# dyustc/CTC-Attention-Mispronunciation

Measured on AMD Instinct MI355X. Metric: phoneme-frames/sec joint CTC-attn decode, 41-phone vocab, higher is better.
Workload: dtype f32 -- reference width (operands with all 24 significand bits, fp32 accumulate; see `accuracy`: closer to a float64 evaluation than ATen's own fp32): the large time-batched contractions (conv0/conv1, BiLSTM and text input projections) run on the bf16 matrix cores as f32x6 = each fp32 operand as thre

## Files before the change

ctc-attention-mispronunciation_amd/csrc/api.hip:

```cpp
#include <stdarg.h>
#include <stdio.h>
#include <string.h>

#include <algorithm>
#include <cmath>
#include <mutex>
#include <vector>

#include "mdd_internal.h"

namespace mdd {

static thread_local char g_err[512] = "";

void set_error(const char *fmt, ...) {
    va_list ap;
    va_start(ap, fmt);
    vsnprintf(g_err, sizeof(g_err), fmt, ap);
    va_end(ap);
}

struct DeviceGate {
    std::mutex mu;
    hipEvent_t done = nullptr;
    hipStream_t stream = nullptr;
    bool armed = false;
};
static DeviceGate g_gate[64];

struct DevBuf {
    float *p = nullptr;
    size_t cap = 0;
};

struct GraphKey {
    const void *x, *x1, *out, *tlen, *llen;
    int B, T, L, Traw;
    bool operator<(const GraphKey &o) const { return memcmp(this, &o, sizeof(GraphKey)) < 0; }
};

}

struct mdd_model {
    mdd_config cfg;
    int device = 0;
    bool finalized = false, taps = false, use_graph = true;
    int precision = 2;
    std::map<std::string, std::vector<float>> host;
    float *w_conv0 = nullptr, *sc0 = nullptr, *sh0 = nullptr;
    float *w_conv1t = nullptr, *sc1 = nullptr, *sh1 = nullptr;
    std::vector<float *> wih, whh, bn_scale, bn_shift;
    float *emb = nullptr, *t_wih = nullptr, *t_whh = nullptr, *t_bias = nullptr;
    float *w_score = nullptr, *fscale = nullptr, *fshift = nullptr, *w_fc = nullptr, *w_fcp = nullptr;
    std::vector<mdd::SplitPtr> wih_s, whh_s;
    std::vector<unsigned short *> wih_3;
    unsigned short *t_wih_3 = nullptr, *w_conv1_3 = nullptr;
    std::vector<unsigned short *> whh_3;
    unsigned short *t_whh_3 = nullptr;
    mdd::SplitPtr t_whh_s{nullptr, nullptr};
    mdd::SplitPtr t_wih_s{nullptr, nullptr}, w_score_s{nullptr, nullptr}, w_conv1_s{nullptr, nullptr};
    std::vector<void *> owned;
    mdd::DevBuf y0, seq0, gx, act[2], xraw, hbuf, cbuf, embo, text, key, S;
    mdd::DevBuf seq0_s, act_s[2], x_s, embo_s, text_s, key_s, hsplit, hx;
    mdd::DevBuf p3;
    std::vector<mdd::DevBuf> tap_rnn;
    int *err_flag = nullptr;
    hipStream_t cap_stream = nullptr;
    int lastB = 0, lastT = 0, lastL = 0;
    int raw_T = 0;
    const int *tlen = nullptr, *llen = nullptr;
    mdd::DevBuf xstack;
    std::map<mdd::GraphKey, hipGraphExec_t> graphs;
    int W1() const { return (cfg.feat + 2 - 3) / 2 + 1; }
    int W2() const { return (W1() + 2 - 3) / 2 + 1; }
    int rnn_in() const { return cfg.channels * W2(); }
    int granule_max_b = 1024;
    bool lstm_persist = true;
    int n_cu = 0;
    unsigned int *sync_words = nullptr;
    bool lstm_x3 = false;
    bool conv_fused() const { return (x3() || x6()) && cfg.feat == 243 && cfg.channels == 32; }
    bool packed_h() const { return cfg.hidden == 384 || cfg.hidden == 256; }
    bool persist(int B) const { return lstm_persist && !lstm_x3 && packed_h() && B <= granule_max_b && (x3() || lstm_persist_f32); }
    bool lstm_persist_f32 = true;
    bool lstm_persist_x6 = true;
    bool lstm_x6_force = false;
    bool lx6(int B) const {
        return x6() && lstm_persist_x6 && persist(B) && B <= mdd::lstm_x6_max_b(cfg.hidden) && (lstm_x6_force || cfg.hidden == 384 || B <= 128);
    }
    bool x6() const {
        return precision == 2 && rnn_in() % 32 == 0 && (2 * cfg.hidden) % 32 == 0 && cfg.emb_dim % 32 == 0;
    }
    bool x3() const {
        return precision == 1 && (cfg.hidden == 384 || cfg.hidden == 256) && rnn_in() % 32 == 0 && cfg.emb_dim % 32 == 0;
    }
};

namespace mdd {

static int upload(mdd_model *m, const std::vector<float> &h, float **dev) {
    MDD_HIP_CHECK(hipMalloc((void **)dev, h.size() * sizeof(float)));
    m->owned.push_back(*dev);
    MDD_HIP_CHECK(hipMemcpy(*dev, h.data(), h.size() * sizeof(float), hipMemcpyHostToDevice));
    return MDD_OK;
}

static unsigned short host_bf16(float x) {
    unsigned u; memcpy(&u, &x, 4);
    u += 0x7FFFu + ((u >> 16) & 1u);
    return (unsigned short)(u >> 16);
}
static float host_bf16_f32(unsigned short b) { unsigned u = (unsigned)b << 16; float f; memcpy(&f, &u, 4); return f; }

static int upload_split(mdd_model *m, const std::vector<float> &h, SplitPtr *out) {
    const size_t n = h.size();
    std::vector<unsigned short> buf(2 * n);
    for (size_t i = 0; i < n; i++) {
        buf[i] = host_bf16(h[i]);
        buf[n + i] = host_bf16(h[i] - host_bf16_f32(buf[i]));
    }
    unsigned short *d = nullptr;
    MDD_HIP_CHECK(hipMalloc((void **)&d, 2 * n * sizeof(unsigned short)));
    m->owned.push_back(d);
    MDD_HIP_CHECK(hipMemcpy(d, buf.data(), 2 * n * sizeof(unsigned short), hipMemcpyHostToDevice));
    out->hi = d; out->lo = d + n;
    return MDD_OK;
}

static SplitPtr split_view(const DevBuf &b, size_t n) {
    SplitPtr s; s.hi = reinterpret_cast<unsigned short *>(b.p); s.lo = s.hi ? s.hi + n : nullptr; return s;
}
static const SplitPtr kNoSplit = {nullptr, nullptr};

static thread_local bool g_ws_moved = false;

static std::mutex g_prep_mu;

static int ensure(DevBuf &b, size_t n, hipStream_t zero_stream) {
    if (b.cap >= n) return MDD_OK;
    g_ws_moved = true;
    if (b.p) MDD_HIP_CHECK(hipFree(b.p));
    b.p = nullptr; b.cap = 0;
    MDD_HIP_CHECK(hipMalloc((void **)&b.p, n * sizeof(float)));
    MDD_HIP_CHECK(hipMemsetAsync(b.p, 0, n * sizeof(float), zero_stream));
    MDD_HIP_CHECK(hipStreamSynchronize(zero_stream));
    b.cap = n;
    return MDD_OK;
}

static const std::vector<float> *get(mdd_model *m, const std::string &key, size_t numel) {
    auto it = m->host.find(key);
    if (it == m->host.end()) { set_error("weight '%s' was never loaded", key.c_str()); return nullptr; }
    if (it->second.size() != numel) {
        set_error("weight '%s' has %zu elements, expected %zu", key.c_str(), it->second.size(), numel);
        return nullptr;
    }
    return &it->second;
}

static bool bn_fold(mdd_model *m, const std::string &prefix, int n, std::vector<float> &scale, std::vector<float> &shift) {
    const auto *w = get(m, prefix + ".weight", n), *b = get(m, prefix + ".bias", n);
    const auto *mu = get(m, prefix + ".running_mean", n), *var = get(m, prefix + ".running_var", n);
    if (!w || !b || !mu || !var) return false;
    scale.resize(n); shift.resize(n);
    for (int i = 0; i < n; i++) {
        scale[i] = (*w)[i] / sqrtf((*var)[i] + m->cfg.bn_eps);
        shift[i] = (*b)[i] - (*mu)[i] * scale[i];
    }
    return true;
}

static bool pack_gate_rows(mdd_model *m, const std::string &base, const char *what, int H, int K, std::vector<float> &out) {
    out.assign((size_t)2 * 4 * H * K, 0.f);
    for (int d = 0; d < 2; d++) {
        const auto *w = get(m, base + what + (d ? "_reverse" : ""), (size_t)4 * H * K);
        if (!w) return false;
        for (int g = 0; g < 4; g++)
            for (int u = 0; u < H; u++)
                memcpy(&out[((size_t)d * 4 * H + u * 4 + g) * K], &(*w)[((size_t)g * H + u) * K], sizeof(float) * K);
    }
    return true;
}

static bool use_packed(const mdd_model *m) { return m->cfg.hidden == 384 || m->cfg.hidden == 256; }

static void pack_whh(const std::vector<float> &w, int H, std::vector<float> &out) {
    const int NUT = H / 4, J = H / 16;
    out.resize(w.size());
    for (int d = 0; d < 2; d++)
        for (int ut = 0; ut < NUT; ut++)
            for (int j = 0; j < J; j++)
                for (int lane = 0; lane < 64; lane++)
                    for (int mm = 0; mm < 4; mm++)
                        out[((((size_t)d * NUT + ut) * J + j) * 64 + lane) * 4 + mm] =
                            w[((size_t)d * 4 * H + ut * 16 + (lane & 15)) * H + 16 * j + 4 * (lane >> 4) + mm];
}

static int upload_split3(mdd_model *m, const std::vector<float> &w, unsigned short **out) {
    const size_t n = w.size();
    std::vector<unsigned short> buf(3 * n);
    for (size_t i = 0; i < n; i++) {
        buf[i] = host_bf16(w[i]);
        const float r1 = w[i] - host_bf16_f32(buf[i]);
        buf[n + i] = host_bf16(r1);
        buf[2 * n + i] = host_bf16(r1 - host_bf16_f32(buf[n + i]));
    }
    MDD_HIP_CHECK(hipMalloc((void **)out, 3 * n * sizeof(unsigned short)));
    m->owned.push_back(*out);
    MDD_HIP_CHECK(hipMemcpy(*out, buf.data(), 3 * n * sizeof(unsigned short), hipMemcpyHostToDevice));
    return MDD_OK;
}

struct Stage { const char *name; int launches; double flops; };

static int n_stages(const mdd_model *m) { return 2 + 2 * m->cfg.layers + 6; }

static int run_stage(mdd_model *m, int si, const float *x, int B, int T, const int64_t *x1, int L, float *logp,
                     hipStream_t st, Stage *info) {
    const mdd_config &c = m->cfg;
    const int H = c.hidden, H2 = 2 * H, G2 = 8 * H, Tp = T / 2, Lp = L, nl = c.layers;
    const bool x3 = m->x3();
    const size_t rows = (size_t)Tp * B, trows = (size_t)L * B;
    static thread_local char namebuf[32];
    Stage dummy; if (!info) info = &dummy;
    info->launches = 1; info->flops = 0.0;
    if (si == 0 && m->conv_fused()) {
        info->name = "conv_fused";
        info->flops = 2.0 * 9 * c.channels * (double)B * Tp * m->W2() * (c.channels + 6.0);
        if (m->x6())
            return launch_conv_fused3(x, m->w_conv0, m->sc0, m->sh0, m->w_conv1_3, m->sc1, m->sh1, reinterpret_cast<unsigned short *>(m->p3.p),
                                      m->taps ? m->seq0.p : nullptr, B, T, m->raw_T, st);
        return launch_conv_fused(x, m->w_conv0, m->sc0, m->sh0, m->w_conv1_s, m->sc1, m->sh1, split_view(m->seq0_s, rows * m->rnn_in()),
                                 nullptr, B, T, m->raw_T, st);
    }
    if (si == 1 && m->conv_fused()) { info->name = "conv1_in_fused"; info->launches = 0; return MDD_OK; }
    if (si == 0) { info->name = "conv0"; info->flops = 2.0 * 9 * c.channels * (double)B * T * m->W1();
        return launch_conv0(x, m->w_conv0, m->sc0, m->sh0, m->y0.p, B, T, c.feat, c.channels, st); }
    if (si == 1) { info->name = "conv1"; info->flops = 2.0 * 9 * c.channels * c.channels * (double)B * Tp * m->W2();
        return launch_conv1(m->y0.p, m->w_conv1t, m->sc1, m->sh1, x3 ? nullptr : m->seq0.p,
                            x3 ? split_view(m->seq0_s, rows * m->rnn_in()) : kNoSplit, B, T, m->W1(), c.channels, st); }
    si -= 2;
    if (si < 2 * nl) {
        const int n = si / 2;
        const int K = n == 0 ? m->rnn_in() : H2;
        if (si % 2 == 0) {
            snprintf(namebuf, sizeof(namebuf), "gemm_ih%d", n); info->name = namebuf;
            info->flops = 2.0 * (double)Tp * B * G2 * K;
            if (x3) {
                const SplitPtr in = n == 0 ? split_view(m->seq0_s, rows * K) : split_view(m->act_s[(n - 1) & 1], rows * K);
                return launch_gemm_bf16x3(in, m->wih_s[n], nullptr, m->gx.p, nullptr, Tp * B, G2, K, K, K, G2, 1, 0, 0, 0, st);
            }
            const float *in = n == 0 ? m->seq0.p : m->act[(n - 1) & 1].p;
            if (m->x6()) {
                unsigned short *p3 = reinterpret_cast<unsigned short *>(m->p3.p);
                if (!(n == 0 && m->conv_fused()))
                    if (int rc = launch_split3(in, Tp * B, K, K, p3, st)) return rc;
                return launch_gemm_f32x6(p3, (size_t)Tp * B * K, m->wih_3[n], (size_t)G2 * K, nullptr, m->gx.p, Tp * B, G2, K, G2, st);
            }
            return launch_gemm_nt(in, m->wih[n], nullptr, m->gx.p, Tp * B, G2, K, K, K, G2, 1, 0, 0, 0, st);
        }
        snprintf(namebuf, sizeof(namebuf), "lstm%d", n); info->name = namebuf;
        info->launches = Tp; info->flops = 2.0 * 2 * (double)B * H * 4 * H * Tp;
        LstmStepArgs a;
        a.gx = m->gx.p; a.whh = m->whh[n]; a.hbuf = m->hbuf.p; a.cbuf = m->cbuf.p;
        a.T = Tp; a.B = B; a.H = H; a.packed = use_packed(m);
        a.whh_split = m->whh_s[n]; a.hsplit = (x3 && m->lstm_x3) ? reinterpret_cast<unsigned short *>(m->hsplit.p) : nullptr;
        a.seqlen = m->tlen;
        if (n == nl - 1) {
            a.out = m->xraw.p; a.out_raw = m->xraw.p; a.oscale = nullptr; a.oshift = nullptr;
            a.out_split = x3 ? split_view(m->x_s, rows * H2) : kNoSplit;
        } else {
            a.out = x3 ? nullptr : m->act[n & 1].p; a.out_raw = m->taps ? m->tap_rnn[n].p : nullptr;
            a.out_split = x3 ? split_view(m->act_s[n & 1], rows * H2) : kNoSplit;
            a.oscale = m->bn_scale[n + 1]; a.oshift = m->bn_shift[n + 1];
        }
        if (m->persist(B)) {
            info->launches = 1;
            if (m->lx6(B)) return launch_lstm_layer_x6(a, m->whh_3[n], reinterpret_cast<unsigned short *>(m->hx.p), m->sync_words, m->err_flag, st);
            return x3 ? launch_lstm_layer_granule(a, reinterpret_cast<unsigned short *>(m->hx.p), m->sync_words, m->err_flag, st)
                      : launch_lstm_layer_f32(a, reinterpret_cast<unsigned short *>(m->hx.p), m->sync_words, m->err_flag, st);
        }
        return launch_lstm_layer(a, st);
    }
    si -= 2 * nl;
    switch (si) {
    case 0:
        info->name = "embed";
        return launch_embed(m->emb, c.emb_rows, c.emb_dim, x1, B, L, x3 ? nullptr : m->embo.p,
                            x3 ? split_view(m->embo_s, trows * c.emb_dim) : kNoSplit, m->err_flag, st);
    case 1:
        info->name = "gemm_text"; info->flops = 2.0 * (double)L * B * G2 * c.emb_dim;
        if (x3) return launch_gemm_bf16x3(split_view(m->embo_s, trows * c.emb_dim), m->t_wih_s, m->t_bias, m->gx.p, nullptr, L * B, G2,
                                          c.emb_dim, c.emb_dim, c.emb_dim, G2, 1, 0, 0, 0, st);
        if (m->x6()) {
            unsigned short *p3 = reinterpret_cast<unsigned short *>(m->p3.p);
            if (int rc = launch_split3(m->embo.p, L * B, c.emb_dim, c.emb_dim, p3, st)) return rc;
            return launch_gemm_f32x6(p3, (size_t)L * B * c.emb_dim, m->t_wih_3, (size_t)G2 * c.emb_dim, m->t_bias, m->gx.p, L * B, G2, c.emb_dim, G2, st);
        }
        return launch_gemm_nt(m->embo.p, m->t_wih, m->t_bias, m->gx.p, L * B, G2, c.emb_dim, c.emb_dim, c.emb_dim, G2, 1, 0, 0, 0, st);
    case 2: {
        info->name = "lstm_text"; info->launches = L; info->flops = 2.0 * 2 * (double)B * H * 4 * H * L;
        LstmStepArgs a;
        a.gx = m->gx.p; a.whh = m->t_whh; a.hbuf = m->hbuf.p; a.cbuf = m->cbuf.p;
        a.out = m->text.p; a.out_raw = m->text.p; a.oscale = nullptr; a.oshift = nullptr;
        a.out_split = x3 ? split_view(m->text_s, trows * H2) : kNoSplit;
        a.T = L; a.B = B; a.H = H; a.packed = use_packed(m);
        a.whh_split = m->t_whh_s; a.hsplit = (x3 && m->lstm_x3) ? reinterpret_cast<unsigned short *>(m->hsplit.p) : nullptr;
        a.seqlen = m->llen;
        if (m->persist(B)) {
            info->launches = 1;
            if (m->lx6(B)) return launch_lstm_layer_x6(a, m->t_whh_3, reinterpret_cast<unsigned short *>(m->hx.p), m->sync_words, m->err_flag, st);
            return x3 ? launch_lstm_layer_granule(a, reinterpret_cast<unsigned short *>(m->hx.p), m->sync_words, m->err_flag, st)
                      : launch_lstm_layer_f32(a, reinterpret_cast<unsigned short *>(m->hx.p), m->sync_words, m->err_flag, st);
        }
// ... 19 lines not shown
}

int device_gate_enter(int device, hipStream_t st, bool *held) {
    *held = false;
    hipStreamCaptureStatus cs = hipStreamCaptureStatusNone;
    if (st && hipStreamIsCapturing(st, &cs) == hipSuccess && cs != hipStreamCaptureStatusNone) return MDD_OK;
    DeviceGate &g = g_gate[device & 63];
    g.mu.lock();
    *held = true;
    if (g.armed && g.stream != st) {
        hipError_t e = hipStreamWaitEvent(st, g.done, 0);
        if (e != hipSuccess) { g.mu.unlock(); *held = false; set_error("device gate: %s", hipGetErrorString(e)); return MDD_ERR_HIP; }
    }
    return MDD_OK;
}
int device_gate_leave(int device, hipStream_t st, bool held, int rc) {
    if (!held) return rc;
    DeviceGate &g = g_gate[device & 63];
    hipError_t e = hipSuccess;
    if (!g.done) e = hipEventCreateWithFlags(&g.done, hipEventDisableTiming);
    if (e == hipSuccess) e = hipEventRecord(g.done, st);
    if (e == hipSuccess) { g.armed = true; g.stream = st; }
    g.mu.unlock();
    if (e != hipSuccess && rc == MDD_OK) { set_error("device gate: %s", hipGetErrorString(e)); return MDD_ERR_HIP; }
    return rc;
}
static int gate_enter(mdd_model *m, hipStream_t st, bool *held) { return device_gate_enter(m->device, st, held); }
static int gate_leave(mdd_model *m, hipStream_t st, bool held, int rc) { return device_gate_leave(m->device, st, held, rc); }

static int forward_enqueue(mdd_model *m, const float *x, int B, int T, const int64_t *x1, int L, float *logp, hipStream_t st) {
    for (int si = 0; si < n_stages(m); si++)
        if (int rc = run_stage(m, si, x, B, T, x1, L, logp, st, nullptr)) return rc;
    return MDD_OK;
}

}

using namespace mdd;

extern "C" const char *mdd_last_error(void) { return g_err; }
extern "C" int mdd_version(void) { return 100; }

extern "C" int mdd_create(const mdd_config *cfg, int device, mdd_model **out) {
    if (!cfg || !out) { set_error("mdd_create: null argument"); return MDD_ERR_ARG; }
    if (cfg->hidden <= 0 || cfg->hidden % 4 || cfg->layers < 1 || cfg->num_class < 2 || cfg->feat < 3 ||
        (cfg->channels != 32 && cfg->channels != 4) || cfg->emb_rows < 1 || cfg->emb_dim < 1) {
        set_error("mdd_create: unsupported geometry (hidden %% 4 == 0, channels in {32,4})");
        return MDD_ERR_ARG;
    }
    int ndev = 0;
    MDD_HIP_CHECK(hipGetDeviceCount(&ndev));
    if (device < 0 || device >= ndev) { set_error("mdd_create: device %d of %d", device, ndev); return MDD_ERR_ARG; }
    MDD_HIP_CHECK(hipSetDevice(device));
    hipDeviceProp_t prop;
    MDD_HIP_CHECK(hipGetDeviceProperties(&prop, device));
    if (strncmp(prop.gcnArchName, "gfx950", 6) != 0) {
        set_error("libmdd_hip is built for gfx950 (MI355X) only; device %d is %s", device, prop.gcnArchName);
        return MDD_ERR_ARG;
    }
    mdd_model *m = new mdd_model();
    m->cfg = *cfg;
    m->device = device;
    const char *pr = getenv("MDD_PRECISION");
    if (pr && (!strcmp(pr, "f32") || !strcmp(pr, "0"))) m->precision = 0;
    if (pr && (!strcmp(pr, "bf16x3") || !strcmp(pr, "1"))) m->precision = 1;
    if (pr && (!strcmp(pr, "f32x6") || !strcmp(pr, "2"))) m->precision = 2;
    const char *lx = getenv("MDD_LSTM");
    m->lstm_x3 = lx && !strcmp(lx, "x3");
    if (lx && !strcmp(lx, "step")) m->lstm_persist = false;
    const char *g = getenv("MDD_GRAPH");
    m->use_graph = !(g && g[0] == '0');
    if (int rc = init_kernel_attributes()) { delete m; return rc; }
    if (int rc = init_lstm_attributes()) { delete m; return rc; }
    if (int rc = init_granule_attributes()) { delete m; return rc; }
    if (int rc = init_lstm_f32_attributes()) { delete m; return rc; }
    if (int rc = init_lstm_x6_attributes()) { delete m; return rc; }
    if (int rc = init_conv_attributes()) { delete m; return rc; }
    if (int rc = init_gemm_attributes()) { delete m; return rc; }
    if (int rc = init_gemm_x6_attributes()) { delete m; return rc; }
    m->n_cu = prop.multiProcessorCount;
    if (!persistent_grid_fits(m->n_cu)) m->lstm_persist = false;
    if (!persistent_f32_grid_fits(m->n_cu)) m->lstm_persist_f32 = false;
    if (!persistent_x6_grid_fits(m->n_cu)) m->lstm_persist_x6 = false;
    { const char *e6 = getenv("MDD_LSTM_X6"); if (e6 && e6[0] == '0') m->lstm_persist_x6 = false; if (e6 && e6[0] == 'f') m->lstm_x6_force = true; }
    hipError_t e = hipMalloc((void **)&m->err_flag, sizeof(int));
    if (e == hipSuccess) e = hipMemset(m->err_flag, 0, sizeof(int));
    if (e == hipSuccess) e = hipStreamCreateWithFlags(&m->cap_stream, hipStreamNonBlocking);
    if (e == hipSuccess) e = hipMalloc((void **)&m->sync_words, 32 * sizeof(unsigned int));
    if (e != hipSuccess) { set_error("mdd_create: %s", hipGetErrorString(e)); delete m; return MDD_ERR_HIP; }
    *out = m;
    return MDD_OK;
}

extern "C" void mdd_destroy(mdd_model *m) {
    if (!m) return;
    (void)hipSetDevice(m->device);
    (void)hipDeviceSynchronize();
    for (auto &kv : m->graphs) (void)hipGraphExecDestroy(kv.second);
    for (void *p : m->owned) (void)hipFree(p);
    DevBuf *bufs[] = {&m->y0, &m->seq0, &m->gx, &m->act[0], &m->act[1], &m->xraw, &m->hbuf, &m->cbuf, &m->embo, &m->text, &m->key, &m->S,
                      &m->seq0_s, &m->act_s[0], &m->act_s[1], &m->x_s, &m->embo_s, &m->text_s, &m->key_s, &m->hsplit, &m->hx, &m->xstack, &m->p3};
    for (DevBuf *b : bufs) if (b->p) (void)hipFree(b->p);
    for (auto &b : m->tap_rnn) if (b.p) (void)hipFree(b.p);
    if (m->err_flag) (void)hipFree(m->err_flag);
    if (m->cap_stream) (void)hipStreamDestroy(m->cap_stream);
    if (m->sync_words) (void)hipFree(m->sync_words);
    delete m;
}

extern "C" int mdd_load_weight(mdd_model *m, const char *key, const float *data, const int64_t *shape, int32_t ndim) {
    if (!m || !key || (!data && ndim > 0) || ndim < 0 || ndim > 4) { set_error("mdd_load_weight: bad argument"); return MDD_ERR_ARG; }
    std::string k(key);
    if (k.size() > 19 && k.compare(k.size() - 19, 19, "num_batches_tracked") == 0) return MDD_OK;
    size_t n = 1;
    for (int i = 0; i < ndim; i++) { if (shape[i] < 0) { set_error("negative dim"); return MDD_ERR_ARG; } n *= (size_t)shape[i]; }
    m->host[k].assign(data, data + n);
    m->finalized = false;
    return MDD_OK;
}

extern "C" int mdd_finalize_weights(mdd_model *m) {
    if (!m) { set_error("null model"); return MDD_ERR_ARG; }
    MDD_HIP_CHECK(hipSetDevice(m->device));
    const mdd_config &c = m->cfg;
    const int ch = c.channels, H = c.hidden;
    int rc;
    for (void *p : m->owned) (void)hipFree(p);
    m->owned.clear(); m->wih.clear(); m->whh.clear(); m->wih_s.clear(); m->whh_s.clear(); m->wih_3.clear(); m->t_wih_3 = nullptr;
    m->bn_scale.assign(c.layers, nullptr); m->bn_shift.assign(c.layers, nullptr);
    for (auto &kv : m->graphs) (void)hipGraphExecDestroy(kv.second);
    m->graphs.clear();
    std::vector<float> sc, sh, tmp;
    {
        const auto *w0 = get(m, "conv.0.conv.weight", (size_t)ch * 9), *b0 = get(m, "conv.0.conv.bias", ch);
        const auto *w1 = get(m, "conv.1.conv.weight", (size_t)ch * ch * 9), *b1 = get(m, "conv.1.conv.bias", ch);
        if (!w0 || !b0 || !w1 || !b1) return MDD_ERR_STATE;
        if (!bn_fold(m, "conv.0.batch_norm", ch, sc, sh)) return MDD_ERR_STATE;
        for (int i = 0; i < ch; i++) sh[i] += (*b0)[i] * sc[i];
        if ((rc = upload(m, *w0, &m->w_conv0)) || (rc = upload(m, sc, &m->sc0)) || (rc = upload(m, sh, &m->sh0))) return rc;
        if (!bn_fold(m, "conv.1.batch_norm", ch, sc, sh)) return MDD_ERR_STATE;
        for (int i = 0; i < ch; i++) sh[i] += (*b1)[i] * sc[i];
        tmp.assign((size_t)ch * 9 * ch, 0.f);
        for (int co = 0; co < ch; co++)
            for (int ci = 0; ci < ch; ci++)
                for (int k = 0; k < 9; k++) tmp[((size_t)ci * 9 + k) * ch + co] = (*w1)[((size_t)co * ch + ci) * 9 + k];
        if ((rc = upload(m, tmp, &m->w_conv1t)) || (rc = upload(m, sc, &m->sc1)) || (rc = upload(m, sh, &m->sh1))) return rc;
        tmp.assign((size_t)ch * 9 * ch, 0.f);
        for (int co = 0; co < ch; co++)
            for (int ci = 0; ci < ch; ci++)
                for (int k = 0; k < 9; k++) tmp[((size_t)co * 9 + k) * ch + ci] = (*w1)[((size_t)co * ch + ci) * 9 + k];
        if ((rc = upload_split(m, tmp, &m->w_conv1_s))) return rc;
        {
            const size_t n = tmp.size();
            std::vector<unsigned short> buf(3 * n);
            for (size_t i = 0; i < n; i++) {
                buf[i] = host_bf16(tmp[i]);
                const float r1 = tmp[i] - host_bf16_f32(buf[i]);
                buf[n + i] = host_bf16(r1);
                buf[2 * n + i] = host_bf16(r1 - host_bf16_f32(buf[n + i]));
            }
            MDD_HIP_CHECK(hipMalloc((void **)&m->w_conv1_3, 3 * n * sizeof(unsigned short)));
            m->owned.push_back(m->w_conv1_3);
            MDD_HIP_CHECK(hipMemcpy(m->w_conv1_3, buf.data(), 3 * n * sizeof(unsigned short), hipMemcpyHostToDevice));
        }
    }
    for (int n = 0; n < c.layers; n++) {
// ... 328 lines not shown
```

ctc-attention-mispronunciation_amd/csrc/frontend.hip:

```cpp
#include "mdd_internal.h"

namespace mdd {

__global__ void stack_skip_kernel(const float *__restrict__ raw, int T_raw, int D, int right, int skip, int kept,
                                  int T_out, float *__restrict__ out) {
    const int W = (right + 1) * D;
    const int b = blockIdx.y, i = blockIdx.x;
    const float *src = raw + (size_t)b * T_raw * D;
    float *dst = out + ((size_t)b * T_out + i) * W;
    for (int j = threadIdx.x; j < W; j += blockDim.x) {
        float v = 0.f;
        if (i < kept) {
            int r = j / D, c = j - r * D;
            int s = i * skip + r;
            if (s > T_raw - 1) s = T_raw - 1;
            v = src[(size_t)s * D + c];
        }
        dst[j] = v;
    }
}

int launch_stack_skip(const float *raw, int B, int T_raw, int D, int right, int skip, int n_down, float *out,
                      hipStream_t st) {
    if (B <= 0 || T_raw <= 0 || D <= 0 || right < 0) { set_error("stack_skip: bad shape"); return MDD_ERR_ARG; }
// ... 259 lines not shown
            }
        }
        __syncthreads();
        f32x16 acc;
#pragma unroll
        for (int r = 0; r < 16; r++) acc[r] = 0.f;
        const int m = min(mt * 32 + li, W2 - 1);
#pragma unroll
        for (int i = 0; i < 9; i++) {
            const int kb = kh2 * 9 + i, kk = kb >> 1, kh = kk / 3, kw = kk - kh * 3;
            const int khs = kh + rot >= 3 ? kh + rot - 3 : kh + rot;
            const int off = (khs * CF_NCOL + 2 * m + kw) * CF_COLB + ((kb & 1) * 16 + half * 8) * 2;
            const bf16x8 ah = *reinterpret_cast<const bf16x8 *>(yh + off);
            const bf16x8 al = *reinterpret_cast<const bf16x8 *>(yl + off);
            if (NP == 3) {
                const bf16x8 am = *reinterpret_cast<const bf16x8 *>(ym + off);
                acc = __builtin_amdgcn_mfma_f32_32x32x16_bf16(am, bwm[i], acc, 0, 0, 0);
                acc = __builtin_amdgcn_mfma_f32_32x32x16_bf16(ah, bwl[i], acc, 0, 0, 0);
                acc = __builtin_amdgcn_mfma_f32_32x32x16_bf16(al, bwh[i], acc, 0, 0, 0);
                acc = __builtin_amdgcn_mfma_f32_32x32x16_bf16(ah, bwm[i], acc, 0, 0, 0);
                acc = __builtin_amdgcn_mfma_f32_32x32x16_bf16(am, bwh[i], acc, 0, 0, 0);
            } else {
                acc = __builtin_amdgcn_mfma_f32_32x32x16_bf16(ah, bwl[i], acc, 0, 0, 0);
                acc = __builtin_amdgcn_mfma_f32_32x32x16_bf16(al, bwh[i], acc, 0, 0, 0);
            }
            acc = __builtin_amdgcn_mfma_f32_32x32x16_bf16(ah, bwh[i], acc, 0, 0, 0);
        }
        if (kh2 == 1) {
#pragma unroll
            for (int r = 0; r < 16; r++) red[mt * 1024 + r * 64 + lane] = acc[r];
        }
        __syncthreads();
        if (kh2 == 0) {
            const float s1 = sc1[li], h1 = sh1[li];
#pragma unroll
            for (int r = 0; r < 16; r++) {
                const int wo = mt * 32 + (r & 3) + 8 * (r >> 2) + 4 * half;
                if (wo < W2) {
                    float v = (acc[r] + red[mt * 1024 + r * 64 + lane]) * s1 + h1;
                    v = v > 0.f ? v : 0.f;
                    __bf16 hb = (__bf16)v;
                    const float r1 = v - (float)hb;
                    oh[li * W2 + wo] = *reinterpret_cast<unsigned short *>(&hb);
                    if (NP == 3) {
                        __bf16 mb = (__bf16)r1, lb = (__bf16)(r1 - (float)mb);
                        om[li * W2 + wo] = *reinterpret_cast<unsigned short *>(&mb);
                        ol[li * W2 + wo] = *reinterpret_cast<unsigned short *>(&lb);
                    } else { __bf16 lb = (__bf16)r1; ol[li * W2 + wo] = *reinterpret_cast<unsigned short *>(&lb); }
                }
            }
        }
        __syncthreads();
        if (NP == 3) {
            const size_t mrows = (size_t)Tp * B;
            if (tid < 244) {
                const size_t dst = (((size_t)(tid >> 2) * mrows + rowid) * 32 + (tid & 3) * 8);
                *reinterpret_cast<u32x4 *>(out_hi + dst) = *reinterpret_cast<const u32x4 *>(oh + tid * 8);
                *reinterpret_cast<u32x4 *>(out_lo + dst) = *reinterpret_cast<const u32x4 *>(om + tid * 8);
                *reinterpret_cast<u32x4 *>(out_lo + mrows * ROW + dst) = *reinterpret_cast<const u32x4 *>(ol + tid * 8);
            }
            if (out_f32)
                for (int i = tid; i < ROW; i += 256)
                    out_f32[(size_t)rowid * ROW + i] = (__uint_as_float((unsigned)oh[i] << 16) + __uint_as_float((unsigned)om[i] << 16)) + __uint_as_float((unsigned)ol[i] << 16);
        } else {
            const size_t base = (size_t)rowid * ROW;
            if (tid < 244) *reinterpret_cast<u32x4 *>(out_hi + base + tid * 8) = *reinterpret_cast<const u32x4 *>(oh + tid * 8);
            else if (tid - 244 < 12) {
                const int q = tid - 244;
                *reinterpret_cast<u32x4 *>(out_lo + base + q * 8) = *reinterpret_cast<const u32x4 *>(ol + q * 8);
            }
            if (tid < 232) {
                const int q = tid + 12;
                *reinterpret_cast<u32x4 *>(out_lo + base + q * 8) = *reinterpret_cast<const u32x4 *>(ol + q * 8);
            }
            if (out_f32)
                for (int i = tid; i < ROW; i += 256)
                    out_f32[base + i] = __uint_as_float((unsigned)oh[i] << 16) + __uint_as_float((unsigned)ol[i] << 16);
        }
    }
}

size_t conv_fused_smem(int np) { return 5 * CF_XLD * 4 + (size_t)np * CF_YPLANE + 2048 * 4 + (size_t)np * 1952 * 2; }

int launch_conv_fused(const float *x, const float *w0, const float *sc0, const float *sh0, SplitPtr w1, const float *sc1,
                      const float *sh1, SplitPtr out, float *out_f32, int B, int T, int Traw, hipStream_t st) {
    const int Tp = T / 2;
    if (Tp <= 0 || B <= 0) return MDD_OK;
    int S = (1024 + B - 1) / B;
    S = S < 1 ? 1 : (S > Tp ? Tp : S);
    const int seg = (Tp + S - 1) / S;
    S = (Tp + seg - 1) / seg;
    hipLaunchKernelGGL(conv_fused_kernel<2>, dim3(B * S), dim3(256), conv_fused_smem(2), st, x, w0, sc0, sh0, w1.hi, w1.lo, sc1, sh1,
                       out.hi, out.lo, out_f32, B, T, Traw, S, seg);
    MDD_LAUNCH_CHECK();
    return MDD_OK;
}

int launch_conv_fused3(const float *x, const float *w0, const float *sc0, const float *sh0, const unsigned short *w1_3, const float *sc1,
                       const float *sh1, unsigned short *out3, float *out_f32, int B, int T, int Traw, hipStream_t st) {
    const int Tp = T / 2;
    if (Tp <= 0 || B <= 0) return MDD_OK;
    int S = (512 + B - 1) / B;
    S = S < 1 ? 1 : (S > Tp ? Tp : S);
    const int seg = (Tp + S - 1) / S;
    S = (Tp + seg - 1) / seg;
    const size_t plane = (size_t)Tp * B * 1952;
    hipLaunchKernelGGL(conv_fused_kernel<3>, dim3(B * S), dim3(256), conv_fused_smem(3), st, x, w0, sc0, sh0, w1_3, w1_3 + 32 * 288, sc1, sh1,
                       out3, out3 + plane, out_f32, B, T, Traw, S, seg);
    MDD_LAUNCH_CHECK();
    return MDD_OK;
}

int init_conv_attributes() {
    MDD_HIP_CHECK(hipFuncSetAttribute((const void *)conv_fused_kernel<2>, hipFuncAttributeMaxDynamicSharedMemorySize, 96 * 1024));
    MDD_HIP_CHECK(hipFuncSetAttribute((const void *)conv_fused_kernel<3>, hipFuncAttributeMaxDynamicSharedMemorySize, 128 * 1024));
    return MDD_OK;
}

}
```

ctc-attention-mispronunciation_amd/csrc/mdd_internal.h:

```cpp
#pragma once
#include <hip/hip_runtime.h>
#include <stdint.h>

#include <map>
#include <string>
#include <vector>

#include "../../include/mdd_hip.h"

namespace mdd {

void set_error(const char *fmt, ...);

#define MDD_HIP_CHECK(expr)                                                                     \
    do {                                                                                        \
        hipError_t e_ = (expr);                                                                 \
        if (e_ != hipSuccess) {                                                                 \
            mdd::set_error("%s failed: %s (%s:%d)", #expr, hipGetErrorString(e_), __FILE__, __LINE__); \
            return MDD_ERR_HIP;                                                                 \
        }                                                                                       \
    } while (0)

#define MDD_LAUNCH_CHECK() MDD_HIP_CHECK(hipGetLastError())

struct SplitPtr { unsigned short *hi, *lo; };

int launch_gemm_nt(const float *A, const float *W, const float *bias, float *C, int M, int N, int K, int lda, int ldw,
                   int ldc, int batch, long sA, long sW, long sC, hipStream_t st);

int launch_gemm_f32(bool ta, bool tb, const float *A, const float *B, const float *bias, float *C, int M, int N, int K, int lda, int ldb,
                    int ldc, int batch, long sA, long sB, long sC, bool accumulate, hipStream_t st, int ksplit = 0);

int launch_gemm_bf16x3(const SplitPtr &A, const SplitPtr &W, const float *bias, float *C, const SplitPtr *Csplit, int M, int N,
                       int K, int lda, int ldw, int ldc, int batch, long sA, long sW, long sC, hipStream_t st);
int init_gemm_attributes();
int launch_split(const float *x, size_t n, const SplitPtr &out, hipStream_t st);
int launch_unsplit(const SplitPtr &in, size_t n, float *x, hipStream_t st);
int launch_split3(const float *x, int rows, int K, int ld, unsigned short *planes, hipStream_t st);
int launch_gemm_f32x6(const unsigned short *A3, size_t a_plane, const unsigned short *W3, size_t w_plane, const float *bias, float *C, int M, int N, int K,
                      int ldc, hipStream_t st, long long *stamps = nullptr);
int init_gemm_x6_attributes();

int launch_stack_skip(const float *raw, int B, int T_raw, int D, int right, int skip, int n_down, float *out,
                      hipStream_t st);
int launch_conv0(const float *x, const float *w, const float *scale, const float *shift, float *y0, int B, int T, int F,
                 int ch, hipStream_t st);
int launch_conv1(const float *y0, const float *w_t, const float *scale, const float *shift, float *seq, SplitPtr seq_split, int B,
                 int T, int W1, int ch, hipStream_t st);

int launch_conv_fused(const float *x, const float *w0, const float *sc0, const float *sh0, SplitPtr w1, const float *sc1,
                      const float *sh1, SplitPtr out, float *out_f32, int B, int T, int Traw, hipStream_t st);
int launch_conv_fused3(const float *x, const float *w0, const float *sc0, const float *sh0, const unsigned short *w1_3, const float *sc1,
                       const float *sh1, unsigned short *out3, float *out_f32, int B, int T, int Traw, hipStream_t st);
int init_conv_attributes();

struct LstmStepArgs {
    const float *gx;
    const float *whh;
    float *hbuf;
    float *cbuf;
    float *out;
    SplitPtr out_split;
    float *out_raw;
    const float *oscale;
    const float *oshift;
    int T, B, H;
    SplitPtr whh_split;
    unsigned short *hsplit;
    int packed;
    float *gates_save = nullptr;
    float *c_save = nullptr;
    const int *seqlen = nullptr;
};
int launch_lstm_layer(const LstmStepArgs &a, hipStream_t st);

int launch_embed(const float *table, int rows, int E, const int64_t *ids, int B, int L, float *out, SplitPtr out_split,
                 int *err_flag, hipStream_t st);
int launch_attn_tail(const float *S, int Lp, const float *X, const float *V, const float *fscale, const float *fshift,
                     const float *wfc, const float *wfcp, float *logp, int Tp, int B, int L, int H2, int C, hipStream_t st,
                     const int *llen = nullptr);

int init_kernel_attributes();
int init_ctc_attributes();
int init_lstm_attributes();
int granule_bg(int B);
int init_granule_attributes();
int persistent_grid_fits(int n_cu);
int launch_lstm_layer_granule(const LstmStepArgs &s, unsigned short *hx, unsigned int *sync, int *err_flag, hipStream_t st);
int launch_zero_fill(void *p, size_t n, hipStream_t st);
int launch_lstm_layer_f32(const LstmStepArgs &s, unsigned short *hx, unsigned int *sync, int *err_flag, hipStream_t st);
int init_lstm_f32_attributes();
int persistent_f32_grid_fits(int n_cu);
int launch_lstm_layer_x6(const LstmStepArgs &s, const unsigned short *whh3, unsigned short *hx, unsigned int *sync, int *err_flag, hipStream_t st);
int init_lstm_x6_attributes();
int persistent_x6_grid_fits(int n_cu);
size_t lstm_x6_hx_bytes(int H, int B);
int lstm_x6_max_b(int H);
size_t lstm_bwd_granule_hx_bytes(int H);
int launch_lstm_bwd_granule(const float *dout, const float *gates, const float *cst, SplitPtr whhT, float *dg, int T, int B, int H, unsigned short *hx,
                            unsigned int *sync, int *err_flag, hipStream_t st);
int device_gate_enter(int device, hipStream_t st, bool *held);
int device_gate_leave(int device, hipStream_t st, bool held, int rc);

}
```

Baseline: 4.188 million.

## Add multi-row fused conv kernel reusing conv0 rows via rotating LDS ring

Adds a new fused conv0+conv1 f32x6 kernel that produces two output time rows per iteration with 512 threads, keeping a rotating ring of conv0 output rows in LDS so overlapping rows are not recomputed. It also prefetches the next input tile into registers while the current tile is computed, and splits the conv1 K reduction across wave groups with an LDS reduction. It becomes the default path for f32x6, with the old row-wise kernel kept behind MDD_CONV=rowwise. The trade-offs are higher LDS and register use with one block per CU, extra barriers, and segment lengths rounded up to a multiple of the row count.

```diff
diff --git a/ctc-attention-mispronunciation_amd/csrc/api.hip b/ctc-attention-mispronunciation_amd/csrc/api.hip
--- a/ctc-attention-mispronunciation_amd/csrc/api.hip
+++ b/ctc-attention-mispronunciation_amd/csrc/api.hip
@@ -85,6 +85,7 @@
     bool lstm_persist_f32 = true;
     bool lstm_persist_x6 = true;
     bool lstm_x6_force = false;
+    bool conv_rowwise = false;
     bool lx6(int B) const {
         return x6() && lstm_persist_x6 && persist(B) && B <= mdd::lstm_x6_max_b(cfg.hidden) && (lstm_x6_force || cfg.hidden == 384 || B <= 128);
     }
@@ -229,7 +230,7 @@
         info->flops = 2.0 * 9 * c.channels * (double)B * Tp * m->W2() * (c.channels + 6.0);
         if (m->x6())
             return launch_conv_fused3(x, m->w_conv0, m->sc0, m->sh0, m->w_conv1_3, m->sc1, m->sh1, reinterpret_cast<unsigned short *>(m->p3.p),
-                                      m->taps ? m->seq0.p : nullptr, B, T, m->raw_T, st);
+                                      m->taps ? m->seq0.p : nullptr, B, T, m->raw_T, st, m->conv_rowwise);
         return launch_conv_fused(x, m->w_conv0, m->sc0, m->sh0, m->w_conv1_s, m->sc1, m->sh1, split_view(m->seq0_s, rows * m->rnn_in()),
                                  nullptr, B, T, m->raw_T, st);
     }
@@ -415,6 +416,7 @@
     if (!persistent_grid_fits(m->n_cu)) m->lstm_persist = false;
     if (!persistent_f32_grid_fits(m->n_cu)) m->lstm_persist_f32 = false;
     if (!persistent_x6_grid_fits(m->n_cu)) m->lstm_persist_x6 = false;
+    { const char *cv = getenv("MDD_CONV"); m->conv_rowwise = cv && !strcmp(cv, "rowwise"); }
     { const char *e6 = getenv("MDD_LSTM_X6"); if (e6 && e6[0] == '0') m->lstm_persist_x6 = false; if (e6 && e6[0] == 'f') m->lstm_x6_force = true; }
     hipError_t e = hipMalloc((void **)&m->err_flag, sizeof(int));
     if (e == hipSuccess) e = hipMemset(m->err_flag, 0, sizeof(int));
diff --git a/ctc-attention-mispronunciation_amd/csrc/frontend.hip b/ctc-attention-mispronunciation_amd/csrc/frontend.hip
--- a/ctc-attention-mispronunciation_amd/csrc/frontend.hip
+++ b/ctc-attention-mispronunciation_amd/csrc/frontend.hip
@@ -365,6 +365,210 @@
 
 size_t conv_fused_smem(int np) { return 5 * CF_XLD * 4 + (size_t)np * CF_YPLANE + 2048 * 4 + (size_t)np * 1952 * 2; }
 
+constexpr int CM_R = 2, CM_NY = 2 * CM_R + 1, CM_NX = 2 * CM_R + 3;
+constexpr int CM_YPLANE = CM_NY * CF_NCOL * 64;
+constexpr int CM_XT = CM_NX * CF_XLD * 4, CM_OST = CM_R * 3 * 1952 * 2;
+constexpr int CM_RED = 2 * CM_R * 16 * 64 * 4;
+constexpr size_t conv_multirow_smem() { return 3 * (size_t)CM_YPLANE + (CM_XT > CM_OST ? CM_XT : CM_OST) + CM_RED + 256; }
+
+__device__ __forceinline__ int cm_yoff(int slot, int col, int chunk) { return (slot * CF_NCOL + col) * 64 + ((chunk ^ ((col >> 2) & 3)) << 4); }
+
+template <int NP, int R>
+__global__ __launch_bounds__(512, 1) void conv_fused_kernel(const float *__restrict__ x, const float *__restrict__ w0,
+                                                            const float *__restrict__ sc0, const float *__restrict__ sh0,
+                                                            const unsigned short *__restrict__ w1_3, const float *__restrict__ sc1,
+                                                            const float *__restrict__ sh1, unsigned short *__restrict__ out3,
+                                                            float *__restrict__ out_f32, int B, int T, int Traw, int S, int seg) {
+    static_assert(NP == 3 && R == CM_R, "multi-row form: f32x6 planes, CM_R rows (LDS layout above)");
+    constexpr int F = 243, W1 = 122, W2 = 61, CH = 32, ROW = CH * W2;
+    constexpr int D0 = F / 3;
+    constexpr int NY = 2 * R + 1, NX = 2 * R + 3;
+    extern __shared__ __attribute__((aligned(16))) unsigned char smem[];
+    unsigned char *yh = smem, *ym = yh + CM_YPLANE, *yl = ym + CM_YPLANE;
+    float *xs = reinterpret_cast<float *>(yl + CM_YPLANE);
+    unsigned short *ost = reinterpret_cast<unsigned short *>(yl + CM_YPLANE);
+    float *red = reinterpret_cast<float *>(yl + CM_YPLANE + (CM_XT > CM_OST ? CM_XT : CM_OST));
+    float *bn0 = red + CM_RED / 4;
+    const int tid = threadIdx.x, lane = tid & 63, wave = tid >> 6;
+    const int li = lane & 31, half = lane >> 5;
+    const int kh2 = wave >> 2, jr = (wave >> 1) & 1, mt = wave & 1;
+    const int Tp = T / 2;
+    const size_t mrows = (size_t)Tp * B;
+
+    bf16x8 bwh[9], bwm[9], bwl[9];
+#pragma unroll
+    for (int i = 0; i < 9; i++) {
+        const size_t o = (size_t)li * 288 + (kh2 * 9 + i) * 16 + half * 8;
+        bwh[i] = *reinterpret_cast<const bf16x8 *>(w1_3 + o);
+        bwm[i] = *reinterpret_cast<const bf16x8 *>(w1_3 + CH * 288 + o);
+        bwl[i] = *reinterpret_cast<const bf16x8 *>(w1_3 + 2 * CH * 288 + o);
+    }
+    bf16x8 w0h, w0m, w0l;
+#pragma unroll
+    for (int j = 0; j < 8; j++) {
+        const int tap = half * 8 + j;
+        const float wv = tap < 9 ? w0[li * 9 + tap] : 0.f;
+        w0h[j] = (__bf16)wv;
+        const float r1 = wv - (float)w0h[j];
+        w0m[j] = (__bf16)r1; w0l[j] = (__bf16)(r1 - (float)w0m[j]);
+    }
+    if (tid < 64) bn0[tid] = tid < 32 ? sc0[tid] : sh0[tid - 32];
+    const float s1 = sc1[li], h1 = sh1[li];
+    for (int i = tid; i < 3 * NY * 16; i += 512) {
+        const int pl = i / (NY * 16), rem = i - pl * (NY * 16);
+        reinterpret_cast<unsigned int *>(smem + pl * CM_YPLANE + (rem >> 4) * CF_NCOL * 64)[rem & 15] = 0u;
+    }
+
+    const int b = blockIdx.x / S, sidx = blockIdx.x - b * S;
+    const int tp_begin = sidx * seg, tp_end = min(Tp, tp_begin + seg);
+    constexpr int XPT = (NX * CF_XLD + 511) / 512;
+    auto load_x = [&](int tp, float (&dst)[XPT]) {
+#pragma unroll
+        for (int k = 0; k < XPT; k++) {
+            const int i = tid + 512 * k, r = i / CF_XLD, c = i - r * CF_XLD - 1, ti = 2 * tp - 2 + r;
+            float v = 0.f;
+            if (i < NX * CF_XLD) {
+                if (Traw == 0) {
+                    if (ti >= 0 && ti < T && c >= 0 && c < F) v = x[((size_t)b * T + ti) * F + c];
+                } else {
+                    const int j = c / D0, fr = min(2 * ti + j, Traw - 1);
+                    if (ti >= 0 && 2 * ti < Traw && c >= 0 && c < F) v = x[((size_t)b * Traw + fr) * D0 + (c - j * D0)];
+                }
+            }
+            dst[k] = v;
+        }
+    };
+    float xnext[XPT];
+    if (tp_begin < tp_end) load_x(tp_begin, xnext);
+    int rot = 0;
+    for (int tp = tp_begin; tp < tp_end; tp += R) {
+        const bool fresh = tp == tp_begin;
+        if (!fresh) rot = rot == 0 ? NY - 1 : rot - 1;
+        __syncthreads();
+#pragma unroll
+        for (int k = 0; k < XPT; k++) if (tid + 512 * k < NX * CF_XLD) xs[tid + 512 * k] = xnext[k];
+        __syncthreads();
+        auto conv0_tile = [&](int p) {
+            const int pc = min(p, NY * W1 - 1);
+            const int r = pc / W1, wc = pc - r * W1, ti = 2 * tp - 1 + r;
+            const int rs = r + rot >= NY ? r + rot - NY : r + rot;
+            const bool inb = p < NY * W1, rowok = ti >= 0 && ti < T && inb;
+            float v[8];
+#pragma unroll
+            for (int j = 0; j < 8; j++) {
+                const int tap = half * 8 + j, kh = tap / 3, kw = tap - kh * 3;
+                v[j] = (tap < 9) ? xs[(r + kh) * CF_XLD + 2 * wc + kw] : 0.f;
+            }
+            bf16x8 bh, bm, bl;
+#pragma unroll
+            for (int j = 0; j < 8; j++) {
+                bh[j] = (__bf16)v[j];
+                const float r1 = v[j] - (float)bh[j];
+                bm[j] = (__bf16)r1; bl[j] = (__bf16)(r1 - (float)bm[j]);
+            }
+            f32x16 d;
+#pragma unroll
+            for (int q = 0; q < 16; q++) d[q] = 0.f;
+            d = __builtin_amdgcn_mfma_f32_32x32x16_bf16(w0m, bm, d, 0, 0, 0);
+            d = __builtin_amdgcn_mfma_f32_32x32x16_bf16(w0h, bl, d, 0, 0, 0);
+            d = __builtin_amdgcn_mfma_f32_32x32x16_bf16(w0l, bh, d, 0, 0, 0);
+            d = __builtin_amdgcn_mfma_f32_32x32x16_bf16(w0h, bm, d, 0, 0, 0);
+            d = __builtin_amdgcn_mfma_f32_32x32x16_bf16(w0m, bh, d, 0, 0, 0);
+            d = __builtin_amdgcn_mfma_f32_32x32x16_bf16(w0h, bh, d, 0, 0, 0);
+            if (inb) {
+#pragma unroll
+                for (int g = 0; g < 4; g++) {
+                    unsigned short hb[4], mb[4], lb[4];
+                    const float4 c0s = *reinterpret_cast<const float4 *>(bn0 + 8 * g + 4 * half);
+                    const float4 c0h = *reinterpret_cast<const float4 *>(bn0 + 32 + 8 * g + 4 * half);
+                    const float cs[4] = {c0s.x, c0s.y, c0s.z, c0s.w}, chh[4] = {c0h.x, c0h.y, c0h.z, c0h.w};
+#pragma unroll
+                    for (int e = 0; e < 4; e++) {
+                        float a = d[4 * g + e] * cs[e] + chh[e];
+                        a = (rowok && a > 0.f) ? a : 0.f;
+                        __bf16 h = (__bf16)a;
+                        const float r1 = a - (float)h;
+                        __bf16 mm_ = (__bf16)r1, l = (__bf16)(r1 - (float)mm_);
+                        hb[e] = *reinterpret_cast<unsigned short *>(&h);
+                        mb[e] = *reinterpret_cast<unsigned short *>(&mm_); lb[e] = *reinterpret_cast<unsigned short *>(&l);
+                    }
+                    const int o = cm_yoff(rs, wc + 1, g) + 8 * half;
+                    *reinterpret_cast<uint2 *>(yh + o) = make_uint2(hb[0] | ((unsigned)hb[1] << 16), hb[2] | ((unsigned)hb[3] << 16));
+                    *reinterpret_cast<uint2 *>(ym + o) = make_uint2(mb[0] | ((unsigned)mb[1] << 16), mb[2] | ((unsigned)mb[3] << 16));
+                    *reinterpret_cast<uint2 *>(yl + o) = make_uint2(lb[0] | ((unsigned)lb[1] << 16), lb[2] | ((unsigned)lb[3] << 16));
+                }
+            }
+        };
+        {
+            const int p0 = fresh ? 0 : W1;
+            conv0_tile(p0 + wave * 32 + li);
+            conv0_tile(p0 + (wave + 8) * 32 + li);
+            if (fresh && wave < 4) conv0_tile((16 + wave) * 32 + li);
+        }
+        if (tp + R < tp_end) load_x(tp + R, xnext);
+        __syncthreads();
+        f32x16 acc;
+#pragma unroll
+        for (int r = 0; r < 16; r++) acc[r] = 0.f;
+        const int m = min(mt * 32 + li, W2 - 1);
+        int slot[3];
+#pragma unroll
+        for (int kh = 0; kh < 3; kh++) { const int r = 2 * jr + kh + rot; slot[kh] = r >= NY ? r - NY : r; }
+#pragma unroll
+        for (int i = 0; i < 9; i++) {
+            const int kb = kh2 * 9 + i, kk = kb >> 1, kh = kk / 3, kw = kk - kh * 3;
+            const int off = cm_yoff(slot[kh], 2 * m + kw, (kb & 1) * 2 + half);
+            const bf16x8 ah = *reinterpret_cast<const bf16x8 *>(yh + off);
+            const bf16x8 am = *reinterpret_cast<const bf16x8 *>(ym + off);
+            const bf16x8 al = *reinterpret_cast<const bf16x8 *>(yl + off);
+            acc = __builtin_amdgcn_mfma_f32_32x32x16_bf16(am, bwm[i], acc, 0, 0, 0);
+            acc = __builtin_amdgcn_mfma_f32_32x32x16_bf16(ah, bwl[i], acc, 0, 0, 0);
+            acc = __builtin_amdgcn_mfma_f32_32x32x16_bf16(al, bwh[i], acc, 0, 0, 0);
+            acc = __builtin_amdgcn_mfma_f32_32x32x16_bf16(ah, bwm[i], acc, 0, 0, 0);
+            acc = __builtin_amdgcn_mfma_f32_32x32x16_bf16(am, bwh[i], acc, 0, 0, 0);
+            acc = __builtin_amdgcn_mfma_f32_32x32x16_bf16(ah, bwh[i], acc, 0, 0, 0);
+        }
+        float *rt = red + (jr * 2 + mt) * 16 * 64;
+        if (kh2 == 1) {
+#pragma unroll
+            for (int r = 0; r < 16; r++) rt[r * 64 + lane] = acc[r];
+        }
+        __syncthreads();
+        if (kh2 == 0 && tp + jr < tp_end) {
+            unsigned short *oh = ost + jr * 3 * ROW, *om = oh + ROW, *ol = om + ROW;
+#pragma unroll
+            for (int r = 0; r < 16; r++) {
+                const int wo = mt * 32 + (r & 3) + 8 * (r >> 2) + 4 * half;
+                if (wo < W2) {
+                    float v = (acc[r] + rt[r * 64 + lane]) * s1 + h1;
+                    v = v > 0.f ? v : 0.f;
+                    __bf16 hb = (__bf16)v;
+                    const float r1 = v - (float)hb;
+                    __bf16 mb = (__bf16)r1, lb = (__bf16)(r1 - (float)mb);
+                    oh[li * W2 + wo] = *reinterpret_cast<unsigned short *>(&hb);
+                    om[li * W2 + wo] = *reinterpret_cast<unsigned short *>(&mb);
+                    ol[li * W2 + wo] = *reinterpret_cast<unsigned short *>(&lb);
+                }
+            }
+        }
+        __syncthreads();
+        const int nr = min(R, tp_end - tp);
+        for (int i = tid; i < nr * 3 * 244; i += 512) {
+            const int jj = i / (3 * 244), rem = i - jj * (3 * 244), pl = rem / 244, q = rem - pl * 244;
+            const size_t rowid = (size_t)(tp + jj) * B + b;
+            unsigned short *dst = out3 + pl * mrows * ROW + ((size_t)(q >> 2) * mrows + rowid) * 32 + (q & 3) * 8;
+            *reinterpret_cast<u32x4 *>(dst) = *reinterpret_cast<const u32x4 *>(ost + (jj * 3 + pl) * ROW + q * 8);
+        }
+        if (out_f32)
+            for (int i = tid; i < nr * ROW; i += 512) {
+                const int jj = i / ROW, c = i - jj * ROW;
+                const unsigned short *oh = ost + jj * 3 * ROW;
+                out_f32[((size_t)(tp + jj) * B + b) * ROW + c] =
+                    (__uint_as_float((unsigned)oh[c] << 16) + __uint_as_float((unsigned)oh[ROW + c] << 16)) + __uint_as_float((unsigned)oh[2 * ROW + c] << 16);
+            }
+    }
+}
+
 int launch_conv_fused(const float *x, const float *w0, const float *sc0, const float *sh0, SplitPtr w1, const float *sc1,
                       const float *sh1, SplitPtr out, float *out_f32, int B, int T, int Traw, hipStream_t st) {
     const int Tp = T / 2;
@@ -380,12 +584,20 @@
 }
 
 int launch_conv_fused3(const float *x, const float *w0, const float *sc0, const float *sh0, const unsigned short *w1_3, const float *sc1,
-                       const float *sh1, unsigned short *out3, float *out_f32, int B, int T, int Traw, hipStream_t st) {
+                       const float *sh1, unsigned short *out3, float *out_f32, int B, int T, int Traw, hipStream_t st, bool rowwise) {
     const int Tp = T / 2;
     if (Tp <= 0 || B <= 0) return MDD_OK;
     int S = (512 + B - 1) / B;
     S = S < 1 ? 1 : (S > Tp ? Tp : S);
-    const int seg = (Tp + S - 1) / S;
+    int seg = (Tp + S - 1) / S;
+    if (!rowwise) {
+        seg = (seg + CM_R - 1) / CM_R * CM_R;
+        S = (Tp + seg - 1) / seg;
+        hipLaunchKernelGGL((conv_fused_kernel<3, CM_R>), dim3(B * S), dim3(512), conv_multirow_smem(), st, x, w0, sc0, sh0, w1_3, sc1, sh1,
+                           out3, out_f32, B, T, Traw, S, seg);
+        MDD_LAUNCH_CHECK();
+        return MDD_OK;
+    }
     S = (Tp + seg - 1) / seg;
     const size_t plane = (size_t)Tp * B * 1952;
     hipLaunchKernelGGL(conv_fused_kernel<3>, dim3(B * S), dim3(256), conv_fused_smem(3), st, x, w0, sc0, sh0, w1_3, w1_3 + 32 * 288, sc1, sh1,
@@ -397,6 +609,7 @@
 int init_conv_attributes() {
     MDD_HIP_CHECK(hipFuncSetAttribute((const void *)conv_fused_kernel<2>, hipFuncAttributeMaxDynamicSharedMemorySize, 96 * 1024));
     MDD_HIP_CHECK(hipFuncSetAttribute((const void *)conv_fused_kernel<3>, hipFuncAttributeMaxDynamicSharedMemorySize, 128 * 1024));
+    MDD_HIP_CHECK(hipFuncSetAttribute((const void *)conv_fused_kernel<3, CM_R>, hipFuncAttributeMaxDynamicSharedMemorySize, (int)conv_multirow_smem()));
     return MDD_OK;
 }
 
diff --git a/ctc-attention-mispronunciation_amd/csrc/mdd_internal.h b/ctc-attention-mispronunciation_amd/csrc/mdd_internal.h
--- a/ctc-attention-mispronunciation_amd/csrc/mdd_internal.h
+++ b/ctc-attention-mispronunciation_amd/csrc/mdd_internal.h
@@ -51,7 +51,8 @@
 int launch_conv_fused(const float *x, const float *w0, const float *sc0, const float *sh0, SplitPtr w1, const float *sc1,
                       const float *sh1, SplitPtr out, float *out_f32, int B, int T, int Traw, hipStream_t st);
 int launch_conv_fused3(const float *x, const float *w0, const float *sc0, const float *sh0, const unsigned short *w1_3, const float *sc1,
-                       const float *sh1, unsigned short *out3, float *out_f32, int B, int T, int Traw, hipStream_t st);
+                       const float *sh1, unsigned short *out3, float *out_f32, int B, int T, int Traw, hipStream_t st,
+                       bool rowwise = false);
 int init_conv_attributes();
 
 struct LstmStepArgs {
```

New measurement: 4.387 million (median of 6 runs). +4.7%, better.
